# bd-iaas-us/infiniStore

Measured on AMD Instinct MI355X. Metric: put_get_GBps, higher is better.
Workload: dtype bf16; 1 GPU; model=kvcache-store, block_kb=128, global_batch=2048, seq_len=0, parallelism=shard1, client_procs=4, resident_steps=976

## Files before the change

### csrc/gpu/gpu.h

```cpp
#pragma once

#include <cstddef>
#include <cstdint>
#include <string>

#include "../core/page_codec.h"

namespace ifs {
namespace gpu {

bool available();
int device_count();
std::string device_name(int dev);
size_t device_total_mem(int dev);

void* alloc_device(int dev, size_t bytes);
void free_device(void* p);
void* alloc_host_pinned(size_t bytes);
void free_host_pinned(void* p);
bool memcpy_d2h(void* dst, const void* src, size_t n);
bool memcpy_h2d(void* dst, const void* src, size_t n);
bool memcpy_d2d(void* dst, const void* src, size_t n);
using Stream = void*;
bool memcpy_h2d_async(void* dst, const void* src, size_t n, Stream s);
bool memcpy_d2h_async(void* dst, const void* src, size_t n, Stream s);
bool memcpy_any_async(void* dst, const void* src, size_t n, Stream s);

constexpr size_t kIpcHandleSize = 64;
struct IpcHandle {
    uint8_t bytes[kIpcHandleSize];
};

bool ipc_export(const void* ptr, IpcHandle* handle, uint64_t* base_offset,
                uint64_t* alloc_size = nullptr);
void* ipc_open(const IpcHandle& handle, int src_device);
bool ipc_close(void* base);

bool enable_peer_access(int dev, int peer);

bool is_device_pointer(const void* ptr);

int export_dmabuf(void* ptr, size_t size, uint64_t* offset);

using Event = void*;
Stream stream_create(int dev);
void stream_destroy(Stream s);
bool stream_sync(Stream s);
Event event_create(int dev);
void event_destroy(Event e);
bool event_record(Event e, Stream s);
bool event_sync(Event e);
bool event_query(Event e);
bool set_device(int dev);

bool launch_copy_blocks(int dev, Stream s, const uint64_t* dev_src_ptrs,
                        const uint64_t* dev_dst_ptrs, int n_blocks, size_t bytes_per_block,
                        bool aligned16, PageSegments seg = {}, PageDir dir = PageDir::kStore);

bool launch_copy_blocks_inline(int dev, Stream s, const uint64_t* src_ptrs,
                               const uint64_t* dst_ptrs, int n_blocks, size_t bytes_per_block);

bool launch_transform_blocks(int dev, Stream s, PageCodec codec, PageDir dir,
                             const uint64_t* dev_src_ptrs, const uint64_t* dev_dst_ptrs,
                             float* dev_scales, int n_blocks, size_t elems_per_block,
                             PageSegments seg = {});
constexpr int kMxfp4GroupsPerIter = 64;

bool launch_load_sliced(int dev, Stream s, PageCodec codec, const uint64_t* dev_src_ptrs,
                        const uint64_t* dev_dst_ptrs, const float* dev_scales, int n_blocks,
                        PageSlice slice, PageSegments seg, bool aligned16);
constexpr int kSliceThreads = 512;

bool launch_hash_blocks(int dev, Stream s, const uint64_t* dev_ptrs, int n_blocks,
                        size_t bytes_per_block, uint64_t* dev_out_hashes);

const char* last_error();

}
}
```

### csrc/gpu/gpu.hip

```cpp
#include "gpu.h"

#include <hip/hip_runtime.h>

#include <atomic>
#include <cstdio>
#include <cstdlib>
#include <cstring>
#include <mutex>

#include "../core/log.h"
#include "fp8_codec.h"
#include "mxfp4_codec.h"

namespace ifs {
namespace gpu {

static thread_local char g_err[256] = {0};
const char* last_error() { return g_err; }

static bool fail(const char* what, hipError_t e) {
    snprintf(g_err, sizeof(g_err), "%s: %s", what, hipGetErrorString(e));
    ERROR("%s", g_err);
    return false;
}
// ... 127 lines not shown
        return nullptr;
    }
    return p;
}

bool ipc_close(void* base) {
    HIP_OK(hipIpcCloseMemHandle(base));
    return true;
}

bool is_device_pointer(const void* ptr) {
    hipPointerAttribute_t attr;
    if (hipPointerGetAttributes(&attr, ptr) != hipSuccess) {
        (void)hipGetLastError();
        return false;
    }
    return attr.type == hipMemoryTypeDevice;
}

int export_dmabuf(void* ptr, size_t size, uint64_t* offset) {
    *offset = 0;
#if HIP_VERSION >= 60000000 || defined(hipMemRangeHandleTypeDmaBufFd)
    int fd = -1;
    hipError_t e = hipMemGetHandleForAddressRange(&fd, reinterpret_cast<hipDeviceptr_t>(ptr),
                                                  size, hipMemRangeHandleTypeDmaBufFd, 0);
    if (e != hipSuccess) {
        fail("hipMemGetHandleForAddressRange", e);
        return -1;
    }
    return fd;
#else
    (void)ptr;
    (void)size;
    return -1;
#endif
}

bool enable_peer_access(int dev, int peer) {
    if (dev == peer) return true;
    int can = 0;
    HIP_OK(hipDeviceCanAccessPeer(&can, dev, peer));
    if (!can) return false;
    HIP_OK(hipSetDevice(dev));
    hipError_t e = hipDeviceEnablePeerAccess(peer, 0);
    if (e != hipSuccess && e != hipErrorPeerAccessAlreadyEnabled) return fail("enable_peer", e);
    return true;
}

Stream stream_create(int dev) {
    if (hipSetDevice(dev) != hipSuccess) return nullptr;
    hipStream_t s = nullptr;
    if (hipStreamCreateWithFlags(&s, hipStreamNonBlocking) != hipSuccess) return nullptr;
    return reinterpret_cast<Stream>(s);
}
void stream_destroy(Stream s) {
    if (s) hipStreamDestroy(reinterpret_cast<hipStream_t>(s));
}
bool stream_sync(Stream s) {
    HIP_OK(hipStreamSynchronize(reinterpret_cast<hipStream_t>(s)));
    return true;
}
Event event_create(int dev) {
    if (hipSetDevice(dev) != hipSuccess) return nullptr;
    hipEvent_t e = nullptr;
    if (hipEventCreateWithFlags(&e, hipEventDisableTiming) != hipSuccess) return nullptr;
    return reinterpret_cast<Event>(e);
}
void event_destroy(Event e) {
    if (e) hipEventDestroy(reinterpret_cast<hipEvent_t>(e));
}
bool event_record(Event e, Stream s) {
    HIP_OK(hipEventRecord(reinterpret_cast<hipEvent_t>(e), reinterpret_cast<hipStream_t>(s)));
    return true;
}
bool event_sync(Event e) {
    HIP_OK(hipEventSynchronize(reinterpret_cast<hipEvent_t>(e)));
    return true;
}
bool event_query(Event e) {
    return hipEventQuery(reinterpret_cast<hipEvent_t>(e)) == hipSuccess;
}



__device__ __forceinline__ uint32_t block_chunk_descs(const uint64_t* __restrict__ src_ptrs,
                                                      const uint64_t* __restrict__ dst_ptrs,
                                                      uint32_t chunks_per_block,
                                                      uint64_t (&sd)[2]) {
    uint32_t b = blockIdx.x / chunks_per_block;
    uint32_t chunk = blockIdx.x - b * chunks_per_block;
    __shared__ uint64_t lds[2];
    if (threadIdx.x == 0) {
        lds[0] = src_ptrs[b];
        lds[1] = dst_ptrs[b];
    }
    __syncthreads();
    sd[0] = lds[0];
    sd[1] = lds[1];
    return chunk;
}

__global__ void copy_blocks_vec_kernel(const uint64_t* __restrict__ src_ptrs,
                                       const uint64_t* __restrict__ dst_ptrs,
                                       uint32_t chunks_per_block,
                                       uint64_t units_per_block) {
    uint64_t sd[2];
    uint32_t chunk = block_chunk_descs(src_ptrs, dst_ptrs, chunks_per_block, sd);
    const uint4* s = reinterpret_cast<const uint4*>(sd[0]);
    uint4* d = reinterpret_cast<uint4*>(sd[1]);
    uint64_t stride = static_cast<uint64_t>(chunks_per_block) * blockDim.x;
    for (uint64_t u = static_cast<uint64_t>(chunk) * blockDim.x + threadIdx.x;
         u < units_per_block; u += stride)
        d[u] = s[u];
}

struct InlineDescs {
    uint64_t src[16];
    uint64_t dst[16];
};

__global__ void copy_blocks_vec_inline_kernel(InlineDescs descs, int n_blocks,
                                              uint64_t units_per_block) {
    uint64_t total = static_cast<uint64_t>(n_blocks) * units_per_block;
    uint64_t stride = static_cast<uint64_t>(gridDim.x) * blockDim.x;
    for (uint64_t u = blockIdx.x * static_cast<uint64_t>(blockDim.x) + threadIdx.x; u < total;
         u += stride) {
        uint64_t b = u / units_per_block;
        uint64_t off = u - b * units_per_block;
        const uint4* s = reinterpret_cast<const uint4*>(descs.src[b]) + off;
        uint4* d = reinterpret_cast<uint4*>(descs.dst[b]) + off;
        *d = *s;
    }
}

bool launch_copy_blocks_inline(int dev, Stream stream, const uint64_t* src_ptrs,
                               const uint64_t* dst_ptrs, int n_blocks, size_t bytes_per_block) {
    if (n_blocks <= 0 || n_blocks > 16 || bytes_per_block % 16 != 0) return false;
    HIP_OK(hipSetDevice(dev));
    hipStream_t s = reinterpret_cast<hipStream_t>(stream);
    InlineDescs descs;
    for (int i = 0; i < n_blocks; i++) {
        descs.src[i] = src_ptrs[i];
        descs.dst[i] = dst_ptrs[i];
    }
    uint64_t upb = bytes_per_block / 16;
    uint64_t total = static_cast<uint64_t>(n_blocks) * upb;
    const int threads = 256;
    int grid = static_cast<int>(std::min<uint64_t>((total + threads - 1) / threads, 4096));
    hipLaunchKernelGGL(copy_blocks_vec_inline_kernel, dim3(grid), dim3(threads), 0, s, descs,
                       n_blocks, upb);
    HIP_OK(hipGetLastError());
    return true;
}

__global__ void copy_blocks_byte_kernel(const uint64_t* __restrict__ src_ptrs,
                                        const uint64_t* __restrict__ dst_ptrs,
                                        uint32_t chunks_per_block,
                                        uint64_t bytes_per_block) {
    uint64_t sd[2];
    uint32_t chunk = block_chunk_descs(src_ptrs, dst_ptrs, chunks_per_block, sd);
    const uint8_t* s = reinterpret_cast<const uint8_t*>(sd[0]);
    uint8_t* d = reinterpret_cast<uint8_t*>(sd[1]);
    uint64_t stride = static_cast<uint64_t>(chunks_per_block) * blockDim.x;
    for (uint64_t u = static_cast<uint64_t>(chunk) * blockDim.x + threadIdx.x;
         u < bytes_per_block; u += stride)
        d[u] = s[u];
}

static uint32_t copy_chunks_per_block(uint64_t units_per_block, uint64_t n_blocks, int threads) {
    uint64_t max_chunks = (units_per_block + threads - 1) / static_cast<uint64_t>(threads);
    uint64_t want = (4096 + n_blocks - 1) / n_blocks;
    uint64_t c = std::min<uint64_t>(std::max<uint64_t>(want, 1), max_chunks);
    return static_cast<uint32_t>(std::max<uint64_t>(c, 1));
}

__device__ __forceinline__ uint32_t block_seg_chunk_descs(const uint64_t* __restrict__ src_ptrs,
                                                          const uint64_t* __restrict__ dst_ptrs,
                                                          uint32_t n_segments,
                                                          uint32_t chunks_per_seg,
                                                          uint64_t (&sd)[2], uint32_t* seg) {
    uint32_t per_block = n_segments * chunks_per_seg;
    uint32_t b = blockIdx.x / per_block;
    uint32_t r = blockIdx.x - b * per_block;
    uint32_t s = r / chunks_per_seg;
    uint32_t chunk = r - s * chunks_per_seg;
    __shared__ uint64_t lds[2];
    if (threadIdx.x == 0) {
        lds[0] = src_ptrs[b];
        lds[1] = dst_ptrs[b];
    }
    __syncthreads();
    sd[0] = lds[0];
    sd[1] = lds[1];
    *seg = s;
    return chunk;
}

__global__ void copy_blocks_vec_seg_kernel(const uint64_t* __restrict__ src_ptrs,
                                           const uint64_t* __restrict__ dst_ptrs,
                                           uint32_t n_segments, uint32_t chunks_per_seg,
                                           uint64_t units_per_seg, uint64_t src_stride,
                                           uint64_t dst_stride) {
    uint64_t sd[2];
    uint32_t seg;
    uint32_t chunk =
        block_seg_chunk_descs(src_ptrs, dst_ptrs, n_segments, chunks_per_seg, sd, &seg);
    const uint4* s = reinterpret_cast<const uint4*>(sd[0] + seg * src_stride);
    uint4* d = reinterpret_cast<uint4*>(sd[1] + seg * dst_stride);
    uint64_t stride = static_cast<uint64_t>(chunks_per_seg) * blockDim.x;
    for (uint64_t u = static_cast<uint64_t>(chunk) * blockDim.x + threadIdx.x;
         u < units_per_seg; u += stride)
        d[u] = s[u];
}

__global__ void copy_blocks_byte_seg_kernel(const uint64_t* __restrict__ src_ptrs,
                                            const uint64_t* __restrict__ dst_ptrs,
                                            uint32_t n_segments, uint32_t chunks_per_seg,
                                            uint64_t bytes_per_seg, uint64_t src_stride,
                                            uint64_t dst_stride) {
    uint64_t sd[2];
    uint32_t seg;
    uint32_t chunk =
        block_seg_chunk_descs(src_ptrs, dst_ptrs, n_segments, chunks_per_seg, sd, &seg);
    const uint8_t* s = reinterpret_cast<const uint8_t*>(sd[0] + seg * src_stride);
    uint8_t* d = reinterpret_cast<uint8_t*>(sd[1] + seg * dst_stride);
    uint64_t stride = static_cast<uint64_t>(chunks_per_seg) * blockDim.x;
    for (uint64_t u = static_cast<uint64_t>(chunk) * blockDim.x + threadIdx.x;
         u < bytes_per_seg; u += stride)
        d[u] = s[u];
}

static bool seg_grid(uint64_t units_per_seg, int n_blocks, uint32_t n_segments, int threads,
                     uint32_t* chunks, uint32_t* grid) {
    uint64_t rows = static_cast<uint64_t>(n_blocks) * n_segments;
    *chunks = copy_chunks_per_block(units_per_seg, rows, threads);
    uint64_t g = rows * *chunks;
    if (g > 0x7fffffffull) return false;
    *grid = static_cast<uint32_t>(g);
    return true;
}

bool launch_copy_blocks(int dev, Stream stream, const uint64_t* dev_src_ptrs,
                        const uint64_t* dev_dst_ptrs, int n_blocks, size_t bytes_per_block,
                        bool aligned16, PageSegments seg, PageDir dir) {
    if (n_blocks <= 0 || bytes_per_block == 0) return true;
    if (!segments_legal(PageCodec::kNone, bytes_per_block, seg.n, seg.stride_bytes)) {
        snprintf(g_err, sizeof(g_err), "launch_copy_blocks: illegal page segments");
        return false;
    }
    HIP_OK(hipSetDevice(dev));
    hipStream_t s = reinterpret_cast<hipStream_t>(stream);
    const int threads = 512;
    if (seg.n > 1) {
        const uint64_t seg_bytes = bytes_per_block / seg.n;
        const bool store = dir == PageDir::kStore;
        const uint64_t src_stride = store ? seg.stride_bytes : seg_bytes;
        const uint64_t dst_stride = store ? seg_bytes : seg.stride_bytes;
        const bool vec = aligned16 && seg_bytes % 16 == 0 && seg.stride_bytes % 16 == 0;
        const uint64_t units = vec ? seg_bytes / 16 : seg_bytes;
        uint32_t chunks, grid;
        if (!seg_grid(units, n_blocks, seg.n, threads, &chunks, &grid)) return false;
        if (vec)
            hipLaunchKernelGGL(copy_blocks_vec_seg_kernel, dim3(grid), dim3(threads), 0, s,
                               dev_src_ptrs, dev_dst_ptrs, seg.n, chunks, units, src_stride,
                               dst_stride);
        else
            hipLaunchKernelGGL(copy_blocks_byte_seg_kernel, dim3(grid), dim3(threads), 0, s,
                               dev_src_ptrs, dev_dst_ptrs, seg.n, chunks, units, src_stride,
                               dst_stride);
        HIP_OK(hipGetLastError());
        return true;
    }
    if (aligned16 && bytes_per_block % 16 == 0) {
        uint64_t upb = bytes_per_block / 16;
        uint32_t chunks = copy_chunks_per_block(upb, n_blocks, threads);
        dim3 grid(static_cast<uint32_t>(n_blocks) * chunks);
        hipLaunchKernelGGL(copy_blocks_vec_kernel, grid, dim3(threads), 0, s, dev_src_ptrs,
                           dev_dst_ptrs, chunks, upb);
    } else {
        uint32_t chunks = copy_chunks_per_block(bytes_per_block, n_blocks, threads);
        dim3 grid(static_cast<uint32_t>(n_blocks) * chunks);
        hipLaunchKernelGGL(copy_blocks_byte_kernel, grid, dim3(threads), 0, s, dev_src_ptrs,
                           dev_dst_ptrs, chunks, bytes_per_block);
    }
    HIP_OK(hipGetLastError());
    return true;
}


__global__ void quant_blocks_bf16_fp8_kernel(const uint64_t* __restrict__ src_ptrs,
                                             const uint64_t* __restrict__ dst_ptrs,
                                             float* __restrict__ scales,
                                             uint64_t elems_per_block) {
    const uint16_t* src = reinterpret_cast<const uint16_t*>(src_ptrs[blockIdx.x]);
    uint8_t* dst = reinterpret_cast<uint8_t*>(dst_ptrs[blockIdx.x]);
    __shared__ uint32_t red[8];
    __shared__ float scale_sh;
    uint32_t m = 0;
    uint64_t n8 = elems_per_block / 8;
    const uint4* src4 = reinterpret_cast<const uint4*>(src);
    for (uint64_t u = threadIdx.x; u < n8; u += blockDim.x) {
        uint4 pk = src4[u];
        const uint16_t* h = reinterpret_cast<const uint16_t*>(&pk);
#pragma unroll
        for (int i = 0; i < 8; i++) m = fp8::absmax_step(m, h[i]);
    }
    for (int off = 32; off; off >>= 1) m = max(m, __shfl_down(m, off, 64));
    if ((threadIdx.x & 63) == 0) red[threadIdx.x >> 6] = m;
    __syncthreads();
    if (threadIdx.x == 0) {
        uint32_t mm = red[0];
        for (int w = 1; w < static_cast<int>(blockDim.x) / 64; w++) mm = max(mm, red[w]);
        scale_sh = fp8::scale_from_absmax_bits(mm);
        scales[blockIdx.x] = scale_sh;
    }
    __syncthreads();
    float inv = 1.f / scale_sh;
    for (uint64_t u = threadIdx.x; u < n8; u += blockDim.x) {
        uint4 pk = src4[u];
        const uint16_t* h = reinterpret_cast<const uint16_t*>(&pk);
        uint8_t out[8];
#pragma unroll
        for (int i = 0; i < 8; i++) {
            float f = fp8::bits_f32(static_cast<uint32_t>(h[i]) << 16);
            out[i] = fp8::f32_to_e4m3(f * inv);
        }
        reinterpret_cast<uint2*>(dst)[u] = *reinterpret_cast<const uint2*>(out);
    }
}

__global__ void dequant_blocks_fp8_bf16_kernel(const uint64_t* __restrict__ src_ptrs,
                                               const uint64_t* __restrict__ dst_ptrs,
                                               const float* __restrict__ scales,
                                               uint64_t elems_per_block) {
    const uint8_t* src = reinterpret_cast<const uint8_t*>(src_ptrs[blockIdx.x]);
    uint16_t* dst = reinterpret_cast<uint16_t*>(dst_ptrs[blockIdx.x]);
    float scale = scales[blockIdx.x];
    uint64_t n8 = elems_per_block / 8;
    for (uint64_t u = threadIdx.x; u < n8; u += blockDim.x) {
        uint2 pk = reinterpret_cast<const uint2*>(src)[u];
        const uint8_t* b = reinterpret_cast<const uint8_t*>(&pk);
        uint16_t out[8];
#pragma unroll
        for (int i = 0; i < 8; i++) out[i] = fp8::decode_to_bf16(b[i], scale);
        reinterpret_cast<uint4*>(dst)[u] = *reinterpret_cast<const uint4*>(out);
    }
}

constexpr int kMxfp4Threads = 4 * kMxfp4GroupsPerIter;

__global__ void quant_blocks_bf16_mxfp4_kernel(const uint64_t* __restrict__ src_ptrs,
                                               const uint64_t* __restrict__ dst_ptrs,
                                               uint32_t chunks_per_block,
                                               uint64_t elems_per_block) {
    uint64_t sd[2];
    uint32_t chunk = block_chunk_descs(src_ptrs, dst_ptrs, chunks_per_block, sd);
    const uint4* src4 = reinterpret_cast<const uint4*>(sd[0]);
    uint32_t* codes = reinterpret_cast<uint32_t*>(sd[1]);
    uint8_t* scales = reinterpret_cast<uint8_t*>(sd[1]) + elems_per_block / 2;
    uint64_t n8 = elems_per_block / 8;
    uint64_t stride = static_cast<uint64_t>(chunks_per_block) * blockDim.x;
    for (uint64_t u = static_cast<uint64_t>(chunk) * blockDim.x + threadIdx.x; u < n8;
         u += stride) {
        uint4 pk = src4[u];
        const uint16_t* h = reinterpret_cast<const uint16_t*>(&pk);
// ... 484 lines not shown
```

### csrc/pybind.cpp

```cpp
#include <pybind11/functional.h>
#include <pybind11/pybind11.h>
#include <pybind11/stl.h>

#include <condition_variable>
#include <memory>
#include <mutex>
#include <thread>

#include "client/client.h"
#include "core/log.h"
#include "fabric/wr_flow.h"
#include "core/protocol.h"
#include "core/mempool.h"
#include "gpu/fp8_codec.h"
#include "gpu/mxfp4_codec.h"
#include "gpu/gpu.h"
#include "server/completed_prefix.h"
#include "server/server.h"

namespace py = pybind11;
using namespace ifs;

namespace {

// ... 150 lines not shown
    if (n == 0) return;
    Pinned<uint64_t> h_src(n), h_dst(n);
    memcpy(h_src.p, src.data(), n * 8);
    memcpy(h_dst.p, dst.data(), n * 8);
    ScopedStream st(device);
    bool ok = inl ? gpu::launch_copy_blocks_inline(device, st.s, h_src.p, h_dst.p,
                                                   static_cast<int>(n), bytes_per_block)
                  : gpu::launch_copy_blocks(device, st.s, h_src.p, h_dst.p,
                                            static_cast<int>(n), bytes_per_block, vec);
    bool synced = gpu::stream_sync(st.s);
    if (!ok || !synced)
        throw std::runtime_error(std::string("_dbg_copy_blocks failed: ") + gpu::last_error());
}

std::vector<float> transform_blocks_py(const char* what, PageCodec codec, PageDir dir,
                                       const std::vector<uint64_t>& src,
                                       const std::vector<uint64_t>& dst,
                                       std::vector<float> scales, size_t elems_per_block,
                                       int device) {
    const PageCodecInfo& info = page_codec_info(codec);
    const bool store = dir == PageDir::kStore;
    require_gpu_and_pairs(what, src, dst);
    if (elems_per_block == 0 || !page_legal(codec, elems_per_block * kPageElemBytes))
        throw std::invalid_argument(std::string(what) + ": elems_per_block % " +
                                    std::to_string(info.page_multiple / kPageElemBytes) +
                                    " != 0");
    if (!all_aligned16(src, dst))
        throw std::invalid_argument(std::string(what) + ": pointers must be 16-byte aligned");
    size_t n = src.size();
    if (info.page_scale && !store && scales.size() != n)
        throw std::invalid_argument(std::string(what) + ": one scale per block");
    scales.resize(info.page_scale ? n : 0);
    if (n == 0) return scales;
    Pinned<uint64_t> h_src(n), h_dst(n);
    Pinned<float> h_scale(n);
    memcpy(h_src.p, src.data(), n * 8);
    memcpy(h_dst.p, dst.data(), n * 8);
    memcpy(h_scale.p, scales.data(), scales.size() * sizeof(float));
    ScopedStream st(device);
    bool ok = gpu::launch_transform_blocks(device, st.s, codec, dir, h_src.p, h_dst.p,
                                           h_scale.p, static_cast<int>(n), elems_per_block);
    bool synced = gpu::stream_sync(st.s);
    if (!ok || !synced)
        throw std::runtime_error(std::string(what) + " failed: " + gpu::last_error());
    memcpy(scales.data(), h_scale.p, scales.size() * sizeof(float));
    return scales;
}


PageCodec codec_from_id(const char* what, int codec) {
    if (codec < 0 || !page_codec_known(static_cast<uint32_t>(codec)))
        throw std::invalid_argument(std::string(what) + ": unknown codec id");
    return static_cast<PageCodec>(codec);
}

void copy_blocks_seg_py(const std::vector<uint64_t>& client, const std::vector<uint64_t>& pool,
                        size_t bytes_per_block, uint32_t n_segments, uint64_t segment_stride,
                        bool to_pool, int device, const std::string& path) {
    const char* what = "_dbg_copy_blocks_seg";
    require_gpu_and_pairs(what, client, pool);
    const bool vec = path == "vec";
    if (!vec && path != "byte")
        throw std::invalid_argument(std::string(what) + ": path must be vec or byte");
    if (bytes_per_block == 0) throw std::invalid_argument(std::string(what) + ": empty blocks");
    if (!segments_legal(PageCodec::kNone, bytes_per_block, n_segments, segment_stride))
        throw std::invalid_argument(std::string(what) + ": illegal page segments");
    if (vec && (bytes_per_block % 16 != 0 || (bytes_per_block / n_segments) % 16 != 0 ||
                (n_segments > 1 && segment_stride % 16 != 0) || !all_aligned16(client, pool)))
        throw std::invalid_argument(std::string(what) +
                                    ": vec path needs 16-byte-aligned pointers, segment size "
                                    "and stride");
    size_t n = client.size();
    if (n == 0) return;
    const std::vector<uint64_t>& src = to_pool ? client : pool;
    const std::vector<uint64_t>& dst = to_pool ? pool : client;
    Pinned<uint64_t> h_src(n), h_dst(n);
    memcpy(h_src.p, src.data(), n * 8);
    memcpy(h_dst.p, dst.data(), n * 8);
    ScopedStream st(device);
    bool ok = gpu::launch_copy_blocks(device, st.s, h_src.p, h_dst.p, static_cast<int>(n),
                                      bytes_per_block, vec,
                                      PageSegments{n_segments, segment_stride},
                                      to_pool ? PageDir::kStore : PageDir::kLoad);
    bool synced = gpu::stream_sync(st.s);
    if (!ok || !synced)
        throw std::runtime_error(std::string(what) + " failed: " + gpu::last_error());
}

std::vector<float> transform_blocks_seg_py(const char* what, int codec_id, PageDir dir,
                                           const std::vector<uint64_t>& src,
                                           const std::vector<uint64_t>& dst,
                                           std::vector<float> scales, size_t elems_per_block,
                                           uint32_t n_segments, uint64_t segment_stride,
                                           int device) {
    const PageCodec codec = codec_from_id(what, codec_id);
    if (!page_codec_transforms(codec))
        throw std::invalid_argument(std::string(what) + ": codec does not transform");
    const PageCodecInfo& info = page_codec_info(codec);
    const bool store = dir == PageDir::kStore;
    require_gpu_and_pairs(what, src, dst);
    if (elems_per_block == 0 || !page_legal(codec, elems_per_block * kPageElemBytes))
        throw std::invalid_argument(std::string(what) + ": illegal page size");
    if (!segments_legal(codec, elems_per_block * kPageElemBytes, n_segments, segment_stride))
        throw std::invalid_argument(std::string(what) + ": illegal page segments");
    if (!all_aligned16(src, dst))
        throw std::invalid_argument(std::string(what) + ": pointers must be 16-byte aligned");
    size_t n = src.size();
    if (info.page_scale && !store && scales.size() != n)
        throw std::invalid_argument(std::string(what) + ": one scale per block");
    scales.resize(info.page_scale ? n : 0);
    if (n == 0) return scales;
    Pinned<uint64_t> h_src(n), h_dst(n);
    Pinned<float> h_scale(n);
    memcpy(h_src.p, src.data(), n * 8);
    memcpy(h_dst.p, dst.data(), n * 8);
    memcpy(h_scale.p, scales.data(), scales.size() * sizeof(float));
    ScopedStream st(device);
    bool ok = gpu::launch_transform_blocks(device, st.s, codec, dir, h_src.p, h_dst.p,
                                           h_scale.p, static_cast<int>(n), elems_per_block,
                                           PageSegments{n_segments, segment_stride});
    bool synced = gpu::stream_sync(st.s);
    if (!ok || !synced)
        throw std::runtime_error(std::string(what) + " failed: " + gpu::last_error());
    memcpy(scales.data(), h_scale.p, scales.size() * sizeof(float));
    return scales;
}

PageSlice slice_from_py(const char* what, const py::object& o, uint64_t unit) {
    PageSlice sl;
    if (o.is_none()) return sl;
    py::tuple t = o.cast<py::tuple>();
    if (t.size() != 5)
        throw std::invalid_argument(std::string(what) +
                                    ": a slice is (n_pieces, page, offset, piece, stride)");
    sl.n = t[0].cast<uint32_t>();
    sl.page_bytes = t[1].cast<uint64_t>() * unit;
    sl.offset = t[2].cast<uint64_t>() * unit;
    sl.piece_bytes = t[3].cast<uint64_t>() * unit;
    sl.stride = t[4].cast<uint64_t>() * unit;
    return sl;
}

bool load_sliced_py(int codec_id, const std::vector<uint64_t>& stored,
                    const std::vector<uint64_t>& client, const std::vector<float>& scales,
                    const py::object& slice, uint32_t n_segments, uint64_t segment_stride,
                    int device) {
    const char* what = "_dbg_load_sliced";
    const PageCodec codec = codec_from_id(what, codec_id);
    const PageSlice sl = slice_from_py(what, slice, 1);
    require_gpu_and_pairs(what, stored, client);
    size_t n = stored.size();
    if (page_codec_info(codec).page_scale && scales.size() != n)
        throw std::invalid_argument(std::string(what) + ": one scale per block");
    if (n == 0) return true;
    py::gil_scoped_release rel;
    Pinned<uint64_t> h_src(n), h_dst(n);
    Pinned<float> h_scale(n);
    memcpy(h_src.p, stored.data(), n * 8);
    memcpy(h_dst.p, client.data(), n * 8);
    memcpy(h_scale.p, scales.data(), std::min(scales.size(), n) * sizeof(float));
    ScopedStream st(device);
    bool ok = gpu::launch_load_sliced(device, st.s, codec, h_src.p, h_dst.p, h_scale.p,
                                      static_cast<int>(n), sl,
                                      PageSegments{n_segments, segment_stride},
                                      all_aligned16(stored, client));
    if (!gpu::stream_sync(st.s))
// ... 469 lines not shown
            "r_rdma_async",
            [](ClientConn& c, const std::vector<std::pair<std::string, uint64_t>>& blocks,
               int block_size, uintptr_t ptr, py::function cb) {
                auto cbp = hold_callback(std::move(cb));
                auto cb_cpp = [cbp]() {
                    py::gil_scoped_acquire acq;
                    (*cbp)();
                };
                py::gil_scoped_release rel;
                return c.r_rdma_async(blocks, block_size, ptr, std::move(cb_cpp));
            })
        .def("sync_rdma", &ClientConn::sync_rdma, py::call_guard<py::gil_scoped_release>())
        .def("check_exist", &ClientConn::check_exist, py::call_guard<py::gil_scoped_release>())
        .def("get_match_last_index", &ClientConn::get_match_last_index,
             py::call_guard<py::gil_scoped_release>())
        .def("delete_keys", &ClientConn::delete_keys, py::call_guard<py::gil_scoped_release>())
        .def("get_stats", &ClientConn::get_stats, py::call_guard<py::gil_scoped_release>())
        .def("shm_active", &ClientConn::shm_active)
        .def("using_verbs", &ClientConn::using_verbs);

    m.def("start_server", &start_server, py::call_guard<py::gil_scoped_release>());
    m.def("stop_server", &stop_server, py::call_guard<py::gil_scoped_release>());
    m.def("purge_kv_map", &purge_kv_map_py);
    m.def("get_kvmap_len", &get_kvmap_len_py);
    m.def("server_stats", &server_stats_py);
    m.def("server_compact", &server_compact_py, py::call_guard<py::gil_scoped_release>());
    m.def("server_snapshot", [](const std::string& path) {
        std::pair<size_t, size_t> r{0, 0};
        bool ok;
        {
            py::gil_scoped_release rel;
            ok = g_server && g_server->snapshot(path, &r);
        }
        return py::make_tuple(ok, r.first, r.second);
    });
    m.def("server_restore", [](const std::string& path) {
        std::pair<size_t, size_t> r{0, 0};
        bool ok;
        {
            py::gil_scoped_release rel;
            ok = g_server && g_server->restore(path, &r);
        }
        return py::make_tuple(ok, r.first, r.second);
    });

    m.def("set_log_level", [](const std::string& lvl) { set_log_level(lvl.c_str()); });
    m.def("log_msg", [](const std::string& lvl, const std::string& msg) {
        LogLevel l = LogLevel::kInfo;
        if (lvl == "debug") l = LogLevel::kDebug;
        else if (lvl == "warning" || lvl == "warn") l = LogLevel::kWarn;
        else if (lvl == "error") l = LogLevel::kError;
        log_printf(l, "python", 0, "%s", msg.c_str());
    });

    m.def("gpu_available", [] { return gpu::available(); });
    m.def("gpu_count", [] { return gpu::device_count(); });
    m.def("hash_blocks", &hash_blocks_py, py::call_guard<py::gil_scoped_release>());

    m.def("_dbg_copy_blocks", &copy_blocks_py, py::arg("src_ptrs"), py::arg("dst_ptrs"),
          py::arg("bytes_per_block"), py::arg("device"), py::arg("path"),
          py::call_guard<py::gil_scoped_release>());
    m.def("_dbg_quant_blocks",
          [](const std::vector<uint64_t>& src, const std::vector<uint64_t>& dst,
             size_t elems_per_block, int device) {
              return transform_blocks_py("_dbg_quant_blocks", PageCodec::kFp8, PageDir::kStore,
                                         src, dst, {}, elems_per_block, device);
          },
          py::arg("src_ptrs"), py::arg("dst_ptrs"), py::arg("elems_per_block"),
          py::arg("device"), py::call_guard<py::gil_scoped_release>());
    m.def("_dbg_dequant_blocks",
          [](const std::vector<uint64_t>& src, const std::vector<uint64_t>& dst,
             const std::vector<float>& scales, size_t elems_per_block, int device) {
              transform_blocks_py("_dbg_dequant_blocks", PageCodec::kFp8, PageDir::kLoad, src,
                                  dst, scales, elems_per_block, device);
          },
          py::arg("src_ptrs"), py::arg("dst_ptrs"), py::arg("scales"),
          py::arg("elems_per_block"), py::arg("device"),
          py::call_guard<py::gil_scoped_release>());

    m.def("_dbg_copy_blocks_seg", &copy_blocks_seg_py, py::arg("client_ptrs"),
          py::arg("pool_ptrs"), py::arg("bytes_per_block"), py::arg("n_segments"),
          py::arg("segment_stride"), py::arg("to_pool"), py::arg("device"), py::arg("path"),
          py::call_guard<py::gil_scoped_release>());
    m.def("_dbg_quant_blocks_seg",
          [](int codec, const std::vector<uint64_t>& src, const std::vector<uint64_t>& dst,
             size_t elems_per_block, uint32_t n_segments, uint64_t segment_stride, int device) {
              return transform_blocks_seg_py("_dbg_quant_blocks_seg", codec, PageDir::kStore,
                                             src, dst, {}, elems_per_block, n_segments,
                                             segment_stride, device);
          },
          py::arg("codec"), py::arg("src_ptrs"), py::arg("dst_ptrs"),
          py::arg("elems_per_block"), py::arg("n_segments"), py::arg("segment_stride"),
          py::arg("device"), py::call_guard<py::gil_scoped_release>());
    m.def("_dbg_dequant_blocks_seg",
          [](int codec, const std::vector<uint64_t>& src, const std::vector<uint64_t>& dst,
             const std::vector<float>& scales, size_t elems_per_block, uint32_t n_segments,
             uint64_t segment_stride, int device) {
              transform_blocks_seg_py("_dbg_dequant_blocks_seg", codec, PageDir::kLoad, src,
                                      dst, scales, elems_per_block, n_segments, segment_stride,
                                      device);
          },
          py::arg("codec"), py::arg("src_ptrs"), py::arg("dst_ptrs"), py::arg("scales"),
          py::arg("elems_per_block"), py::arg("n_segments"), py::arg("segment_stride"),
          py::arg("device"), py::call_guard<py::gil_scoped_release>());

    m.def("_dbg_page_codec", &page_codec_py, py::arg("flags"), py::arg("page_bytes"));
    m.def("_dbg_segments_legal",
          [](int codec, size_t page_bytes, uint64_t n_segments, uint64_t stride_bytes) {
              return segments_legal(codec_from_id("_dbg_segments_legal", codec), page_bytes,
                                    n_segments, stride_bytes);
          },
          py::arg("codec"), py::arg("page_bytes"), py::arg("n_segments"),
          py::arg("stride_bytes"));
    m.attr("_MAX_PAGE_SEGMENTS") = kMaxPageSegments;
    m.def("_dbg_slice_legal",
          [](int codec, const py::object& slice, uint32_t n_segments, uint64_t stride_bytes) {
              if (slice.is_none())
                  throw std::invalid_argument("_dbg_slice_legal: a slice is a tuple of 5");
              return slice_legal(codec_from_id("_dbg_slice_legal", codec),
                                 slice_from_py("_dbg_slice_legal", slice, 1),
                                 PageSegments{n_segments, stride_bytes});
          },
          py::arg("codec"), py::arg("slice"), py::arg("n_segments") = 1,
          py::arg("stride_bytes") = 0);
    m.attr("_MAX_SLICE_PIECES") = kMaxSlicePieces;
    m.attr("_SLICE_THREADS") = gpu::kSliceThreads;
    m.def("_dbg_load_sliced", &load_sliced_py, py::arg("codec"), py::arg("stored_ptrs"),
          py::arg("client_ptrs"), py::arg("scales"), py::arg("slice"),
          py::arg("n_segments") = 1, py::arg("segment_stride") = 0, py::arg("device") = 0);
    m.def("_dbg_shard_run_sliced",
          [](int device, int n_streams, int slots_per_stream, size_t max_descs_per_slot,
             const py::list& copy_jobs, const py::list& slices, int n_threads,
             double timeout_s) -> py::object {
              py::tuple out = shard_run_impl("_dbg_shard_run_sliced", device, n_streams,
                                             slots_per_stream, max_descs_per_slot, copy_jobs,
                                             py::list(), n_threads, timeout_s, &slices);
              return out[0];
          },
          py::arg("device"), py::arg("n_streams"), py::arg("slots_per_stream"),
          py::arg("max_descs_per_slot"), py::arg("copy_jobs"), py::arg("slices"),
          py::arg("n_threads"), py::arg("timeout_s"));
    m.def("_dbg_shard_run", &shard_run_py, py::arg("device"), py::arg("n_streams"),
          py::arg("slots_per_stream"), py::arg("max_descs_per_slot"), py::arg("copy_jobs"),
          py::arg("fabric_jobs"), py::arg("n_threads"), py::arg("timeout_s"));
    m.attr("_SHARD_FAN_CHUNK") = Shard::kFanChunk;
    m.attr("_FAB_STAGE_BYTES") = Shard::kFabStageBytes;
    m.attr("_FAB_STAGE_DESCS") = Shard::kFabStageDescs;
    m.def("_dbg_completed_prefix", &completed_prefix_py, py::arg("has_slot"),
          py::arg("fired_at_query"));
    m.def("_dbg_build_packed_local",
          [](int device, int pid, uint64_t base_ptr, uint64_t base_offset, uint32_t block_size,
             uint32_t flags, uint32_t alloc_mb, py::bytes ipc,
             const std::vector<uint64_t>& offsets, const std::vector<std::string>& keys,
             uint32_t n_segments, uint64_t segment_stride, const py::object& slice) {
              const PackedLocalSliceExt sl =
                  slice_to_wire(slice_from_py("_dbg_build_packed_local", slice, 1));
              std::string ipc_s = ipc;
              if (ipc_s.size() != 64)
                  throw std::invalid_argument("_dbg_build_packed_local: ipc is 64 bytes");
              if (offsets.size() != keys.size())
                  throw std::invalid_argument("_dbg_build_packed_local: one offset per key");
              PackedLocalHdr h;
              h.device = device;
              h.pid = pid;
              h.base_ptr = base_ptr;
              h.base_offset = base_offset;
              h.block_size = block_size;
              h.n_blocks = static_cast<uint32_t>(keys.size());
              h.flags = flags;
              h.rsvd = alloc_mb;
              memcpy(h.ipc, ipc_s.data(), 64);
              std::string blob;
              for (size_t i = 0; i < keys.size(); i++) {
                  if (i) blob.push_back('\0');
                  blob.append(keys[i]);
              }
              auto v = build_packed_local(h, n_segments, segment_stride, offsets.data(),
                                          blob.data(), blob.size(), &sl);
              return py::bytes(reinterpret_cast<const char*>(v.data()), v.size());
          },
          py::arg("device"), py::arg("pid"), py::arg("base_ptr"), py::arg("base_offset"),
          py::arg("block_size"), py::arg("flags"), py::arg("alloc_mb"), py::arg("ipc"),
          py::arg("offsets"), py::arg("keys"), py::arg("n_segments") = 1,
          py::arg("segment_stride") = 0, py::arg("slice") = py::none());
    m.def("_dbg_parse_packed_local", [](const std::string& op, py::bytes data) {
        std::string s = data;
        PackedLocalReq r;
        if (op != "w" && op != "r")
            throw std::invalid_argument("_dbg_parse_packed_local: op is \"w\" or \"r\"");
        if (!parse_packed_local(op[0], reinterpret_cast<const uint8_t*>(s.data()), s.size(), &r))
            throw std::invalid_argument("_dbg_parse_packed_local: INVALID_REQ");
        py::dict d;
        d["device"] = r.hdr.device;
        d["pid"] = r.hdr.pid;
        d["base_ptr"] = r.hdr.base_ptr;
        d["base_offset"] = r.hdr.base_offset;
        d["block_size"] = r.hdr.block_size;
        d["flags"] = r.hdr.flags;
        d["alloc_mb"] = r.hdr.rsvd;
        d["n_segments"] = r.n_segments;
        d["segment_stride"] = r.segment_stride;
        if (r.slice.n_pieces)
            d["slice"] = py::make_tuple(r.slice.n_pieces, r.slice.page_bytes, r.slice.offset,
                                        r.slice.piece_bytes, r.slice.stride);
        else
            d["slice"] = py::none();
        py::list offs, keys;
        for (auto& [key, off] : r.blocks) {
            offs.append(off);
// ... 304 lines not shown
```

Baseline: 2201 GB/s.

## Replace per-chunk copy grid with persistent CU-sized walk using nontemporal 64B-per-thread copies

The vectorised block-copy kernels (plain and segmented) now run on a persistent grid of about 8 workgroups per CU. Each workgroup walks items of 256 threads x 4 uint4 loads, batching 64 descriptor lookups into LDS per pass. Loads and stores use nontemporal builtins, and the CU count is cached per device. The aim is to cut launch and scheduling overhead from a huge grid of small workgroups, raise the number of memory ops in flight per thread, and avoid cache pollution. The tradeoff is fewer resident waves and extra index arithmetic, and the grid sizing might underfill the memory pipeline for some block sizes.

```diff
diff --git a/csrc/gpu/gpu.h b/csrc/gpu/gpu.h
--- a/csrc/gpu/gpu.h
+++ b/csrc/gpu/gpu.h
@@ -55,7 +55,11 @@
 
 bool launch_copy_blocks(int dev, Stream s, const uint64_t* dev_src_ptrs,
                         const uint64_t* dev_dst_ptrs, int n_blocks, size_t bytes_per_block,
-                        bool aligned16, PageSegments seg = {}, PageDir dir = PageDir::kStore);
+                        bool aligned16, PageSegments seg = {}, PageDir dir = PageDir::kStore,
+                        uint32_t max_workgroups = 0);
+constexpr int kCopyThreads = 256;
+constexpr int kCopyLoads = 4;
+constexpr uint32_t kCopyItemUnits = kCopyThreads * kCopyLoads;
 
 bool launch_copy_blocks_inline(int dev, Stream s, const uint64_t* src_ptrs,
                                const uint64_t* dst_ptrs, int n_blocks, size_t bytes_per_block);
diff --git a/csrc/gpu/gpu.hip b/csrc/gpu/gpu.hip
--- a/csrc/gpu/gpu.hip
+++ b/csrc/gpu/gpu.hip
@@ -233,6 +233,75 @@
 }
 
 
+constexpr int kCopyWgPerCu = 8;
+constexpr uint32_t kCopyDescBatch = 64;
+
+typedef uint32_t u32x4 __attribute__((ext_vector_type(4)));
+typedef const __attribute__((address_space(1))) u32x4* GlobalSrc16;
+typedef __attribute__((address_space(1))) u32x4* GlobalDst16;
+
+__device__ __forceinline__ void copy_item(uint64_t src, uint64_t dst, uint64_t left) {
+    GlobalSrc16 s = (GlobalSrc16)src + threadIdx.x;
+    GlobalDst16 d = (GlobalDst16)dst + threadIdx.x;
+    if (left >= kCopyItemUnits) {
+        u32x4 v[kCopyLoads];
+#pragma unroll
+        for (int k = 0; k < kCopyLoads; k++)
+            v[k] = __builtin_nontemporal_load(s + k * kCopyThreads);
+#pragma unroll
+        for (int k = 0; k < kCopyLoads; k++)
+            __builtin_nontemporal_store(v[k], d + k * kCopyThreads);
+    } else {
+#pragma nounroll
+        for (uint32_t o = 0; o + threadIdx.x < left; o += kCopyThreads)
+            __builtin_nontemporal_store(__builtin_nontemporal_load(s + o), d + o);
+    }
+}
+
+template <bool kSegmented>
+__device__ __forceinline__ void copy_walk(const uint64_t* __restrict__ src_ptrs,
+                                          const uint64_t* __restrict__ dst_ptrs,
+                                          uint32_t n_items, uint32_t chunks, uint64_t units,
+                                          uint32_t n_segments, uint64_t src_stride,
+                                          uint64_t dst_stride) {
+    __shared__ uint64_t lds[2][kCopyDescBatch];
+    const uint32_t G = gridDim.x;
+    const uint32_t per_block = kSegmented ? n_segments * chunks : chunks;
+    for (uint64_t first = blockIdx.x; first < n_items;
+         first += static_cast<uint64_t>(kCopyDescBatch) * G) {
+        const uint32_t f = static_cast<uint32_t>(first);
+        const uint32_t mine = (n_items - f + G - 1) / G;
+        const uint32_t cnt = mine < kCopyDescBatch ? mine : kCopyDescBatch;
+        if (f != blockIdx.x) __syncthreads();
+        if (threadIdx.x < cnt) {
+            uint32_t b = (f + threadIdx.x * G) / per_block;
+            uint64_t s0 = src_ptrs[b], d0 = dst_ptrs[b];
+            lds[0][threadIdx.x] = s0;
+            lds[1][threadIdx.x] = d0;
+        }
+        __syncthreads();
+        uint32_t it = f;
+#pragma nounroll
+        for (uint32_t j = 0; j < cnt; j++, it += G) {
+            uint32_t r = it - (it / per_block) * per_block;
+            uint64_t s0 = lds[0][j], d0 = lds[1][j];
+            if (kSegmented) {
+                uint32_t sg = r / chunks;
+                r -= sg * chunks;
+                s0 += sg * src_stride;
+                d0 += sg * dst_stride;
+            }
+            uint64_t u0 = static_cast<uint64_t>(r) * kCopyItemUnits;
+            copy_item(s0 + u0 * 16, d0 + u0 * 16, units - u0);
+        }
+    }
+}
+
+__global__ __launch_bounds__(kCopyThreads, 8) void copy_blocks_vec_kernel(
+    const uint64_t* __restrict__ src_ptrs, const uint64_t* __restrict__ dst_ptrs,
+    uint32_t n_items, uint32_t chunks_per_block, uint64_t units_per_block) {
+    copy_walk<false>(src_ptrs, dst_ptrs, n_items, chunks_per_block, units_per_block, 1, 0, 0);
+}
 
 __device__ __forceinline__ uint32_t block_chunk_descs(const uint64_t* __restrict__ src_ptrs,
                                                       const uint64_t* __restrict__ dst_ptrs,
@@ -241,28 +310,11 @@
     uint32_t b = blockIdx.x / chunks_per_block;
     uint32_t chunk = blockIdx.x - b * chunks_per_block;
     __shared__ uint64_t lds[2];
-    if (threadIdx.x == 0) {
-        lds[0] = src_ptrs[b];
-        lds[1] = dst_ptrs[b];
-    }
+    if (threadIdx.x < 2) lds[threadIdx.x] = (threadIdx.x ? dst_ptrs : src_ptrs)[b];
     __syncthreads();
     sd[0] = lds[0];
     sd[1] = lds[1];
     return chunk;
-}
-
-__global__ void copy_blocks_vec_kernel(const uint64_t* __restrict__ src_ptrs,
-                                       const uint64_t* __restrict__ dst_ptrs,
-                                       uint32_t chunks_per_block,
-                                       uint64_t units_per_block) {
-    uint64_t sd[2];
-    uint32_t chunk = block_chunk_descs(src_ptrs, dst_ptrs, chunks_per_block, sd);
-    const uint4* s = reinterpret_cast<const uint4*>(sd[0]);
-    uint4* d = reinterpret_cast<uint4*>(sd[1]);
-    uint64_t stride = static_cast<uint64_t>(chunks_per_block) * blockDim.x;
-    for (uint64_t u = static_cast<uint64_t>(chunk) * blockDim.x + threadIdx.x;
-         u < units_per_block; u += stride)
-        d[u] = s[u];
 }
 
 struct InlineDescs {
@@ -336,10 +388,7 @@
     uint32_t s = r / chunks_per_seg;
     uint32_t chunk = r - s * chunks_per_seg;
     __shared__ uint64_t lds[2];
-    if (threadIdx.x == 0) {
-        lds[0] = src_ptrs[b];
-        lds[1] = dst_ptrs[b];
-    }
+    if (threadIdx.x < 2) lds[threadIdx.x] = (threadIdx.x ? dst_ptrs : src_ptrs)[b];
     __syncthreads();
     sd[0] = lds[0];
     sd[1] = lds[1];
@@ -347,21 +396,12 @@
     return chunk;
 }
 
-__global__ void copy_blocks_vec_seg_kernel(const uint64_t* __restrict__ src_ptrs,
-                                           const uint64_t* __restrict__ dst_ptrs,
-                                           uint32_t n_segments, uint32_t chunks_per_seg,
-                                           uint64_t units_per_seg, uint64_t src_stride,
-                                           uint64_t dst_stride) {
-    uint64_t sd[2];
-    uint32_t seg;
-    uint32_t chunk =
-        block_seg_chunk_descs(src_ptrs, dst_ptrs, n_segments, chunks_per_seg, sd, &seg);
-    const uint4* s = reinterpret_cast<const uint4*>(sd[0] + seg * src_stride);
-    uint4* d = reinterpret_cast<uint4*>(sd[1] + seg * dst_stride);
-    uint64_t stride = static_cast<uint64_t>(chunks_per_seg) * blockDim.x;
-    for (uint64_t u = static_cast<uint64_t>(chunk) * blockDim.x + threadIdx.x;
-         u < units_per_seg; u += stride)
-        d[u] = s[u];
+__global__ __launch_bounds__(kCopyThreads, 8) void copy_blocks_vec_seg_kernel(
+    const uint64_t* __restrict__ src_ptrs, const uint64_t* __restrict__ dst_ptrs,
+    uint32_t n_items, uint32_t n_segments, uint32_t chunks_per_seg, uint64_t units_per_seg,
+    uint64_t src_stride, uint64_t dst_stride) {
+    copy_walk<true>(src_ptrs, dst_ptrs, n_items, chunks_per_seg, units_per_seg, n_segments,
+                    src_stride, dst_stride);
 }
 
 __global__ void copy_blocks_byte_seg_kernel(const uint64_t* __restrict__ src_ptrs,
@@ -391,9 +431,46 @@
     return true;
 }
 
+static int cached_cu_count(int dev) {
+    constexpr int kMaxDevices = 64;
+    static std::atomic<int> cus[kMaxDevices];
+    const bool cacheable = dev >= 0 && dev < kMaxDevices;
+    int n = cacheable ? cus[dev].load(std::memory_order_relaxed) : 0;
+    if (n > 0) return n;
+    if (hipDeviceGetAttribute(&n, hipDeviceAttributeMultiprocessorCount, dev) != hipSuccess ||
+        n <= 0)
+        return 0;
+    if (cacheable) cus[dev].store(n, std::memory_order_relaxed);
+    return n;
+}
+
+static bool walk_grid(int dev, uint64_t rows, uint64_t units, uint32_t max_workgroups,
+                      uint32_t* chunks, uint32_t* n_items, uint32_t* grid) {
+    uint64_t c = (units + kCopyItemUnits - 1) / kCopyItemUnits;
+    uint64_t items = rows * c;
+    if (c > 0x7fffffffull || items > 0x7fffffffull || max_workgroups > 0x7fffffffu) {
+        snprintf(g_err, sizeof(g_err), "launch_copy_blocks: request too large for one launch");
+        return false;
+    }
+    *chunks = static_cast<uint32_t>(c);
+    *n_items = static_cast<uint32_t>(items);
+    if (max_workgroups) {
+        *grid = max_workgroups;
+        return true;
+    }
+    int cus = cached_cu_count(dev);
+    if (cus <= 0) {
+        snprintf(g_err, sizeof(g_err), "launch_copy_blocks: no CU count for device %d", dev);
+        return false;
+    }
+    *grid = static_cast<uint32_t>(
+        std::min<uint64_t>(items, static_cast<uint64_t>(kCopyWgPerCu) * cus));
+    return true;
+}
+
 bool launch_copy_blocks(int dev, Stream stream, const uint64_t* dev_src_ptrs,
                         const uint64_t* dev_dst_ptrs, int n_blocks, size_t bytes_per_block,
-                        bool aligned16, PageSegments seg, PageDir dir) {
+                        bool aligned16, PageSegments seg, PageDir dir, uint32_t max_workgroups) {
     if (n_blocks <= 0 || bytes_per_block == 0) return true;
     if (!segments_legal(PageCodec::kNone, bytes_per_block, seg.n, seg.stride_bytes)) {
         snprintf(g_err, sizeof(g_err), "launch_copy_blocks: illegal page segments");
@@ -402,36 +479,40 @@
     HIP_OK(hipSetDevice(dev));
     hipStream_t s = reinterpret_cast<hipStream_t>(stream);
     const int threads = 512;
+    uint32_t chunks, n_items, grid;
     if (seg.n > 1) {
         const uint64_t seg_bytes = bytes_per_block / seg.n;
         const bool store = dir == PageDir::kStore;
         const uint64_t src_stride = store ? seg.stride_bytes : seg_bytes;
         const uint64_t dst_stride = store ? seg_bytes : seg.stride_bytes;
         const bool vec = aligned16 && seg_bytes % 16 == 0 && seg.stride_bytes % 16 == 0;
-        const uint64_t units = vec ? seg_bytes / 16 : seg_bytes;
-        uint32_t chunks, grid;
-        if (!seg_grid(units, n_blocks, seg.n, threads, &chunks, &grid)) return false;
-        if (vec)
-            hipLaunchKernelGGL(copy_blocks_vec_seg_kernel, dim3(grid), dim3(threads), 0, s,
-                               dev_src_ptrs, dev_dst_ptrs, seg.n, chunks, units, src_stride,
+        if (vec) {
+            const uint64_t units = seg_bytes / 16;
+            if (!walk_grid(dev, static_cast<uint64_t>(n_blocks) * seg.n, units, max_workgroups,
+                           &chunks, &n_items, &grid))
+                return false;
+            hipLaunchKernelGGL(copy_blocks_vec_seg_kernel, dim3(grid), dim3(kCopyThreads), 0, s,
+                               dev_src_ptrs, dev_dst_ptrs, n_items, seg.n, chunks, units,
+                               src_stride, dst_stride);
+        } else {
+            if (!seg_grid(seg_bytes, n_blocks, seg.n, threads, &chunks, &grid)) return false;
+            hipLaunchKernelGGL(copy_blocks_byte_seg_kernel, dim3(grid), dim3(threads), 0, s,
+                               dev_src_ptrs, dev_dst_ptrs, seg.n, chunks, seg_bytes, src_stride,
                                dst_stride);
-        else
-            hipLaunchKernelGGL(copy_blocks_byte_seg_kernel, dim3(grid), dim3(threads), 0, s,
-                               dev_src_ptrs, dev_dst_ptrs, seg.n, chunks, units, src_stride,
-                               dst_stride);
+        }
         HIP_OK(hipGetLastError());
         return true;
     }
     if (aligned16 && bytes_per_block % 16 == 0) {
         uint64_t upb = bytes_per_block / 16;
-        uint32_t chunks = copy_chunks_per_block(upb, n_blocks, threads);
-        dim3 grid(static_cast<uint32_t>(n_blocks) * chunks);
-        hipLaunchKernelGGL(copy_blocks_vec_kernel, grid, dim3(threads), 0, s, dev_src_ptrs,
-                           dev_dst_ptrs, chunks, upb);
+        if (!walk_grid(dev, n_blocks, upb, max_workgroups, &chunks, &n_items, &grid))
+            return false;
+        hipLaunchKernelGGL(copy_blocks_vec_kernel, dim3(grid), dim3(kCopyThreads), 0, s,
+                           dev_src_ptrs, dev_dst_ptrs, n_items, chunks, upb);
     } else {
-        uint32_t chunks = copy_chunks_per_block(bytes_per_block, n_blocks, threads);
-        dim3 grid(static_cast<uint32_t>(n_blocks) * chunks);
-        hipLaunchKernelGGL(copy_blocks_byte_kernel, grid, dim3(threads), 0, s, dev_src_ptrs,
+        chunks = copy_chunks_per_block(bytes_per_block, n_blocks, threads);
+        dim3 bgrid(static_cast<uint32_t>(n_blocks) * chunks);
+        hipLaunchKernelGGL(copy_blocks_byte_kernel, bgrid, dim3(threads), 0, s, dev_src_ptrs,
                            dev_dst_ptrs, chunks, bytes_per_block);
     }
     HIP_OK(hipGetLastError());
diff --git a/csrc/pybind.cpp b/csrc/pybind.cpp
--- a/csrc/pybind.cpp
+++ b/csrc/pybind.cpp
@@ -256,6 +256,41 @@
                                       bytes_per_block, vec,
                                       PageSegments{n_segments, segment_stride},
                                       to_pool ? PageDir::kStore : PageDir::kLoad);
+    bool synced = gpu::stream_sync(st.s);
+    if (!ok || !synced)
+        throw std::runtime_error(std::string(what) + " failed: " + gpu::last_error());
+}
+
+void copy_blocks_walk_py(const std::vector<uint64_t>& src, const std::vector<uint64_t>& dst,
+                         size_t bytes_per_block, int device, const std::string& path,
+                         uint32_t max_workgroups, uint32_t segments, uint64_t segment_stride,
+                         bool to_pool) {
+    const char* what = "_dbg_copy_blocks_walk";
+    require_gpu_and_pairs(what, src, dst);
+    const bool vec = path == "vec";
+    if (!vec && path != "byte")
+        throw std::invalid_argument(std::string(what) + ": path must be vec or byte");
+    if (bytes_per_block == 0) throw std::invalid_argument(std::string(what) + ": empty blocks");
+    if (max_workgroups > (1u << 20))
+        throw std::invalid_argument(std::string(what) + ": max_workgroups above 2^20");
+    if (!segments_legal(PageCodec::kNone, bytes_per_block, segments, segment_stride))
+        throw std::invalid_argument(std::string(what) + ": illegal page segments");
+    if (vec && (bytes_per_block % 16 != 0 || (bytes_per_block / segments) % 16 != 0 ||
+                (segments > 1 && segment_stride % 16 != 0) || !all_aligned16(src, dst)))
+        throw std::invalid_argument(std::string(what) +
+                                    ": vec path needs 16-byte-aligned pointers, (segment) "
+                                    "size and stride");
+    size_t n = src.size();
+    if (n == 0) return;
+    Pinned<uint64_t> h_src(n), h_dst(n);
+    memcpy(h_src.p, src.data(), n * 8);
+    memcpy(h_dst.p, dst.data(), n * 8);
+    ScopedStream st(device);
+    bool ok = gpu::launch_copy_blocks(device, st.s, h_src.p, h_dst.p, static_cast<int>(n),
+                                      bytes_per_block, vec,
+                                      PageSegments{segments, segment_stride},
+                                      to_pool ? PageDir::kStore : PageDir::kLoad,
+                                      max_workgroups);
     bool synced = gpu::stream_sync(st.s);
     if (!ok || !synced)
         throw std::runtime_error(std::string(what) + " failed: " + gpu::last_error());
@@ -891,6 +926,10 @@
           py::arg("pool_ptrs"), py::arg("bytes_per_block"), py::arg("n_segments"),
           py::arg("segment_stride"), py::arg("to_pool"), py::arg("device"), py::arg("path"),
           py::call_guard<py::gil_scoped_release>());
+    m.def("_dbg_copy_blocks_walk", &copy_blocks_walk_py, py::arg("src_ptrs"),
+          py::arg("dst_ptrs"), py::arg("bytes_per_block"), py::arg("device"), py::arg("path"),
+          py::arg("max_workgroups"), py::arg("segments") = 1, py::arg("segment_stride") = 0,
+          py::arg("to_pool") = true, py::call_guard<py::gil_scoped_release>());
     m.def("_dbg_quant_blocks_seg",
           [](int codec, const std::vector<uint64_t>& src, const std::vector<uint64_t>& dst,
              size_t elems_per_block, uint32_t n_segments, uint64_t segment_stride, int device) {
@@ -934,6 +973,9 @@
           py::arg("stride_bytes") = 0);
     m.attr("_MAX_SLICE_PIECES") = kMaxSlicePieces;
     m.attr("_SLICE_THREADS") = gpu::kSliceThreads;
+    m.attr("_COPY_THREADS") = gpu::kCopyThreads;
+    m.attr("_COPY_LOADS") = gpu::kCopyLoads;
+    m.attr("_COPY_ITEM_UNITS") = gpu::kCopyItemUnits;
     m.def("_dbg_load_sliced", &load_sliced_py, py::arg("codec"), py::arg("stored_ptrs"),
           py::arg("client_ptrs"), py::arg("scales"), py::arg("slice"),
           py::arg("n_segments") = 1, py::arg("segment_stride") = 0, py::arg("device") = 0);
```

New measurement: 2397 GB/s (median of 6 runs). 1.09x the previous value.
